# courtois-neuromod/phantom_vlb

Measured on AMD Instinct MI355X. Metric: clips/sec fine-tune VideoLLaMA2-7B+LoRA->2k-voxel head, 1/2/4/8 MI355X, higher is better.
Workload: dtype bf16; 1 GPU; configs[2]: VideoLLaMA2-7B + LoRA r=16 + 2k-voxel head, bf16; clips_per_gpu=3, global_batch=3, seq_len=2048, frames=12, num_target=2048, weights=random-init, comm=none

## Files before the change

include/vlb.h:

```cpp
#ifndef VLB_H
#define VLB_H

#include <stdint.h>

#ifdef __cplusplus
extern "C" {
#endif
#if defined(__GNUC__) || defined(__clang__)
#pragma GCC visibility push(default)
#endif

#define VLB_OK 0
#define VLB_ERR_INVALID (-1)
#define VLB_ERR_LAUNCH (-2)

#define VLB_ABI_VERSION 2

#define VLB_ACT_NONE 0
#define VLB_ACT_QUICK_GELU 1
#define VLB_ACT_GELU 2
#define VLB_ACT_SILU 3
#define VLB_ACT_SWIGLU_PAIR 4
#define VLB_ACT_SWIGLU_BWD 5

// ... 80 lines not shown
                 float* d_ridge_w, float* d_ridge_b, float* d_ln2_w, float* d_ln2_b, float* d_ln1_w, float* d_ln1_b,
                 float* ws, float* dz_ws, float* dpooled_ws, void* dhidden, int B, int S, int E, int V, float eps,
                 float l2_lambda, float loss_scale, float l2_scale, const int* cu_rows, int total_rows, void* stream);

int vlb_feature_cache_store(const float* pooled_raw, const float* sumw, const int32_t* rows, float* cache_pooled,
                            float* cache_sumw, int B, int E, int n_rows, void* stream);
int vlb_head_fwd_cached(const float* cache_pooled, const float* cache_sumw, const int32_t* rows, const void* ln1_w,
                        const void* ln1_b, const void* ln2_w, const void* ln2_b, const void* ridge_w, const void* ridge_b,
                        const float* y, const float* keep_scale, float* ws, float* pooled_raw, float* sumw, float* zhat,
                        float* ln2_rstd, void* z, float* pred, float* loss_terms, int B, int E, int V, int n_rows, float eps,
                        float l2_lambda, void* stream);
int vlb_head_bwd_cached(const void* ln1_w, const void* ln2_w, const void* ridge_w, const float* y, const float* keep_scale,
                        const float* pooled_raw, const float* sumw, const float* zhat, const float* ln2_rstd, const void* z,
                        const float* pred, float* d_ridge_w, float* d_ridge_b, float* d_ln2_w, float* d_ln2_b, float* d_ln1_w,
                        float* d_ln1_b, float* ws, float* dz_ws, float* dpooled_ws, int B, int E, int V, float eps,
                        float l2_lambda, float loss_scale, float l2_scale, void* stream);

int vlb_lora_down(const void* x, int ldx, const void* A, void* t, int ldt, int M, int K, int R, float scale,
                  float drop_p, const uint32_t* seeds_host, void* stream);
int vlb_lora_merge(const void* W, int ldw, void* Wm, int ldwm, const void* Bt, const void* A, int N, int K, int R, float scale,
                   int row_map, void* stream);
int vlb_lora_dx_masked(const void* u, int ldu, const void* At, int ldat, void* dx, int lddx, int M, int K, int R, float drop_p,
                       const uint32_t* seeds_host, void* stream);
int64_t vlb_wgrad_u_ws_floats(int M, int K);
int vlb_wgrad_skinny_u(const void* G, int ldg, const void* X, int ldx, float* dW, float* ws, int M, int K, float alpha,
                       float beta, const void* Bt, float u_scale, void* u, int ldu, float* u_ws, void* stream);
int vlb_wgrad_skinny_u_multi(const void* G, int ldg, const void* X, int ldx, int M, int nproj, const int* cols, float* const* dW,
                             const void* const* Bt, float* ws, float alpha, float beta, float u_scale, void* u, int ldu,
                             float* u_ws, void* stream);
int vlb_transpose16_scatter(const void* jobs, int n_jobs, void* stream);
int vlb_wgrad_splits(int M);
int vlb_wgrad_skinny(const void* G, int ldg, const void* X, int ldx, float* dW, float* ws, int M, int N, int K,
                     float alpha, float beta, float drop_p, const uint32_t* seeds_host, void* stream);

int vlb_sumsq_ws_floats(void);
int vlb_grad_sumsq(const float* g, int64_t n, float* sumsq, float* ws, void* stream);
int vlb_adamw_step(float* master, void* param_bf16, const float* grad, float* m, float* v, int64_t n, float lr,
                   float beta1, float beta2, float eps, float weight_decay, int step, const float* sumsq,
                   float max_norm, void* stream);
int vlb_grad_accum(float* acc, const float* g, int64_t n, int first, float* sumsq, float* ws, void* stream);
int vlb_grad_accum_bf16(float* acc, const void* g_bf16, int64_t n, int first, float* sumsq, float* ws, void* stream);

int vlb_transpose_pad(const void* in, int ld_in, void* out, int ld_out, int R, int C, int Rpad, void* stream);
int64_t vlb_norm_bwd_ws_floats(int rows, int dim);
int64_t vlb_colsum_ws_floats(int rows, int dim);
int vlb_rmsnorm_bwd_dw(const void* x, const void* dy, void* dw_bf16, float* ws, int rows, int dim, float eps, void* stream);
int64_t vlb_rmsnorm_bwd_full_ws_floats(int rows, int dim);
int vlb_rmsnorm_bwd_full(const void* x, const void* w, const void* dy, const void* dx_in, void* dx, void* dw_bf16, float* ws,
                         int rows, int dim, float eps, void* stream);
int vlb_layernorm_bwd(const void* x, const void* w, const void* b, const void* residual, const void* dy, void* dx, void* dres,
                      void* dw_bf16, void* db_bf16, float* ws, int rows, int dim, float eps, int act, void* stream);
int vlb_act_fwd(const void* x, void* y, int64_t n, int act, void* stream);
int vlb_act_bwd(const void* x, const void* dy, void* dx, int64_t n, int act, void* stream);
int vlb_colsum(const void* x, int ld, void* out_bf16, float* ws, int rows, int dim, void* stream);
int vlb_embed_grad(const void* d_embeds, int ld, const int* tok, const int* beg, const int* rows, int n_tokens, void* dE, int D,
                   void* stream);
int vlb_grad_sumsq_bf16(const void* g, int64_t n, float* sumsq, float* ws, void* stream);
int vlb_adamw_step_g16(float* master, void* param_bf16, const void* grad_bf16, float* m, float* v, int64_t n, float lr,
                       float beta1, float beta2, float eps, float weight_decay, int step, const float* sumsq, float max_norm,
                       void* stream);
int64_t vlb_dwconv3x3_bwd_w_ws_floats(int N, int H, int C);
int vlb_dwconv3x3_bwd_w(const void* x, const void* dy, void* dw9_bf16, float* ws, int N, int H, int W, int C, void* stream);
int vlb_se_bwd_gate(const void* x, const void* dy, const void* s, void* ds, int N, int HW, int C, void* stream);
int vlb_se_bwd_x(const void* dy, const void* s, const void* dpool, void* dx, int N, int HW, int C, void* stream);
int vlb_col2im3d_k2s2p1(const void* dcols, void* dx, int B, int T, int H, int W, int C, void* stream);

// ... 45 lines not shown
```

phantom_vlb_amd/_lib.py:

```python
from __future__ import annotations

import ctypes
import os
from ctypes import c_char_p, c_double, c_float, c_int, c_int64, c_void_p

import torch

_HERE = os.path.dirname(os.path.abspath(__file__))
LIB_PATH = os.environ.get("VLB_LIB") or os.path.join(_HERE, "libvlb.so")
IS_PRODUCT_LIB = os.path.abspath(LIB_PATH) == os.path.join(_HERE, "libvlb.so")

P, I, F, L = c_void_p, c_int, c_float, c_int64

SIGNATURES = {
    "vlb_abi_version": [],
    "vlb_last_error": [],
    "vlb_gemm_bf16": [P, I, P, I, P, I, I, I, I, P, P, I, I, P, I, P, I, I, P],
    "vlb_gemm_bf16_ws": [P, I, P, I, P, I, I, I, I, P, P, I, I, P, I, P, I, I, P, L, P],
    "vlb_gemm_swiglu_save": [P, I, P, I, P, I, P, I, I, I, I, P, I, P, I, I, P, L, P],
    "vlb_gemm_workspace_bytes": [],
    "vlb_gemm_plan": [I, I, I, I, I],
    "vlb_gemm_kernel_choice": [I, I, I, I],
    "vlb_transpose_bf16": [P, P, I, I, P],
    "vlb_attention_fwd": [P, I, P, I, P, I, P, I, P, P, I, I, I, I, I, I, F, P, P],
    "vlb_attention_bwd": [P, I, P, I, P, I, P, I, P, I, P, P, P, I, P, I, P, I, P, P, I, I, I, I, I, I, F, P, I, P],
    "vlb_rmsnorm_fwd": [P, P, P, I, I, F, P],
    "vlb_rmsnorm_bwd": [P, P, P, P, P, I, I, F, P],
    "vlb_layernorm_fwd": [P, P, P, P, P, I, I, F, I, P],
    "vlb_rope_inplace": [P, I, P, P, I, I, I, I, I, P, P],
    "vlb_swiglu_fwd": [P, P, I, I, P],
    "vlb_swiglu_bwd": [P, P, P, I, I, P],
    "vlb_add_bf16": [P, P, P, L, P],
    "vlb_patchify": [P, P, I, I, I, I, I, P],
    "vlb_vit_assemble": [P, P, P, P, I, I, I, P],
    "vlb_drop_cls": [P, P, I, I, I, P],
    "vlb_dwconv3x3": [P, P, P, I, I, I, I, P],
    "vlb_se_pool": [P, P, I, I, I, P],
    "vlb_se_scale": [P, P, P, I, I, I, P],
    "vlb_im2col3d_k2s2p1": [P, P, I, I, I, I, I, P],
    "vlb_splice_embed": [P, P, P, P, P, P, I, I, I, I, L, I, P, P, P],
    "vlb_weight_mask": [P, P, P, P, I, I, I, I, I, I, P],
    "vlb_head_partial_rows": [I],
    "vlb_head_ws_floats": [I, I, I, I],
    "vlb_head_fwd": [P] * 19 + [I, I, I, I, F, F, P, P],
    "vlb_head_bwd": [P] * 24 + [I, I, I, I, F, F, F, F, P, I, P],
    "vlb_feature_cache_store": [P] * 5 + [I, I, I, P],
    "vlb_head_fwd_cached": [P] * 19 + [I, I, I, I, F, F, P],
    "vlb_head_bwd_cached": [P] * 20 + [I, I, I, F, F, F, F, P],
    "vlb_gemm_bf16_masked_pair": [P, I, P, I, P, I, I, I, I, P, I, P, I, F, ctypes.c_uint32, P],
    "vlb_gemm_masked_pair_swiglu_bwd": [P, I, P, I, P, I, P, I, I, I, I, P, I, P, I, F, ctypes.c_uint32, P, L, P],
    "vlb_gemm_bf16_masked_pair_ws": [P, I, P, I, P, I, I, I, I, P, I, P, I, F, ctypes.c_uint32, P, L, P],
    "vlb_wgrad_u_ws_floats": [I, I],
    "vlb_wgrad_skinny_u": [P, I, P, I, P, P, I, I, F, F, P, F, P, I, P, P],
    "vlb_wgrad_skinny_u_multi": [P, I, P, I, I, I, P, P, P, P, F, F, F, P, I, P, P],
    "vlb_transpose16_scatter": [P, I, P],
    "vlb_wgrad_splits": [I],
    "vlb_wgrad_skinny": [P, I, P, I, P, P, I, I, I, F, F, F, P, P],
    "vlb_lora_down": [P, I, P, P, I, I, I, I, F, F, P, P],
    "vlb_lora_merge": [P, I, P, I, P, P, I, I, I, F, I, P],
    "vlb_lora_dx_masked": [P, I, P, I, P, I, I, I, I, F, P, P],
    "vlb_sumsq_ws_floats": [],
    "vlb_grad_sumsq": [P, L, P, P, P],
    "vlb_adamw_step": [P, P, P, P, P, L, F, F, F, F, F, I, P, F, P],
    "vlb_grad_accum": [P, P, L, I, P, P, P],
    "vlb_grad_accum_bf16": [P, P, L, I, P, P, P],
    "vlb_dropout_keep_scale": [P, L, F, ctypes.c_uint32, P],
    "vlb_transpose_pad": [P, I, P, I, I, I, I, P],
    "vlb_norm_bwd_ws_floats": [I, I],
    "vlb_colsum_ws_floats": [I, I],
    "vlb_rmsnorm_bwd_dw": [P, P, P, P, I, I, F, P],
    "vlb_rmsnorm_bwd_full_ws_floats": [I, I],
    "vlb_rmsnorm_bwd_full": [P, P, P, P, P, P, P, I, I, F, P],
    "vlb_layernorm_bwd": [P, P, P, P, P, P, P, P, P, P, I, I, F, I, P],
    "vlb_act_fwd": [P, P, L, I, P],
    "vlb_act_bwd": [P, P, P, L, I, P],
    "vlb_colsum": [P, I, P, P, I, I, P],
    "vlb_embed_grad": [P, I, P, P, P, I, P, I, P],
    "vlb_grad_sumsq_bf16": [P, L, P, P, P],
    "vlb_adamw_step_g16": [P, P, P, P, P, L, F, F, F, F, F, I, P, F, P],
    "vlb_dwconv3x3_bwd_w_ws_floats": [I, I, I],
    "vlb_dwconv3x3_bwd_w": [P, P, P, P, I, I, I, I, P],
    "vlb_se_bwd_gate": [P, P, P, P, I, I, I, P],
    "vlb_se_bwd_x": [P, P, P, P, I, I, I, P],
    "vlb_col2im3d_k2s2p1": [P, P, I, I, I, I, I, P],
    "vlb_quantize_mxfp8": [P, I, P, I, P, I, I, I, P],
    "vlb_transpose_quantize_mxfp8": [P, I, P, I, P, I, I, I, I, P],
    "vlb_quantize_dual_mxfp8": [P, I, P, I, P, I, P, I, P, I, I, I, I, P],
    "vlb_rmsnorm_fwd_mxfp8": [P, P, P, P, I, P, I, I, I, F, P],
    "vlb_swiglu_fwd_mxfp8": [P, P, P, I, P, I, I, I, P],
    "vlb_gemm_mxfp8": [P, I, P, I, P, I, P, I, P, I, I, I, I, P, I, P],
# ... 55 lines not shown
```

phantom_vlb_amd/csrc/lora.hip:

```cpp
#include "common.hpp"

namespace {

__device__ __forceinline__ uint32_t lowbias32(uint32_t x) {
  x ^= x >> 16; x *= 0x7feb352dU; x ^= x >> 15; x *= 0x846ca68bU; x ^= x >> 16;
  return x;
}
__device__ __forceinline__ uint32_t drop_bits_pair(uint32_t seed, int64_t m, int K, int kpair) {
  const uint64_t c = (uint64_t)m * (uint64_t)(K >> 1) + (uint64_t)kpair;
  return lowbias32((uint32_t)c ^ lowbias32((uint32_t)(c >> 32) + seed));
}
__device__ __forceinline__ uint32_t drop_bits_fast(uint32_t key, uint32_t row_base, int kpair) {
  return lowbias32((row_base + (uint32_t)kpair) ^ key);
}

struct Seeds { uint32_t s[8]; uint32_t key[8]; uint32_t fast; };

__device__ __forceinline__ uint32_t drop_bits(const Seeds& sd, int g, int64_t m, int K, int kpair) {
  return sd.fast ? drop_bits_fast(sd.key[g], (uint32_t)m * (uint32_t)(K >> 1), kpair) : drop_bits_pair(sd.s[g], m, K, kpair);
}
__device__ __forceinline__ void keep8(const Seeds& sd, int g, int64_t m, int K, int k0, uint32_t thresh, bool (&keep)[8]) {
#pragma unroll
  for (int q = 0; q < 4; ++q) {
    const uint32_t h = drop_bits(sd, g, m, K, (k0 >> 1) + q);
// ... 126 lines not shown
        }
#pragma unroll
        for (int e = 0; e < 4; ++e) sum[4 * t + e] += d[e] * inv_keep;
      }
    }
    if (live) {
      bf16x8 o0, o1;
#pragma unroll
      for (int e = 0; e < 8; ++e) {
        o0[e] = (bf16)((float)old0[e] + sum[e]);
        o1[e] = (bf16)((float)old1[e] + sum[8 + e]);
      }
      *reinterpret_cast<bf16x8*>(prow + kcol) = o0;
      *reinterpret_cast<bf16x8*>(prow + kcol + 8) = o1;
    }
    old0 = nx0; old1 = nx1;
  }
}

constexpr int WG_COLS = 256;
constexpr int WG_STEP = 32;

typedef short s16x4_t __attribute__((ext_vector_type(4)));
typedef short s16x8_t __attribute__((ext_vector_type(8)));

__device__ __forceinline__ void glds16_l(const void* g, void* l) {
  __builtin_amdgcn_global_load_lds((const void __attribute__((address_space(1)))*)g,
                                   (void __attribute__((address_space(3)))*)l, 16, 0, 0);
}
__device__ __forceinline__ int xsw(int r) { return (r & 3) | (((r >> 3) & 1) << 2); }

struct UProj { int col0[4]; const bf16* bt[3]; float* dW[3]; int n; };

template <int G, bool WITH_U = false>
__global__ __launch_bounds__(256) void wgrad_mfma_kernel(const bf16* __restrict__ Gm, int ldg, const bf16* __restrict__ X,
                                                         int ldx, float* __restrict__ ws, int M, int K,
                                                         int rows_per_split, uint32_t thresh, Seeds seeds,
                                                         UProj up = UProj{}, float* __restrict__ upart = nullptr) {
  constexpr int XT = WG_STEP * WG_COLS * 2;
  constexpr int GT = WG_STEP * 16 * G * 2;
  constexpr int UT = WITH_U ? 2 * 4 * 2 * 4 * 64 * 4 : 0;
  __shared__ __attribute__((aligned(16))) char smem[2 * (XT + GT) + UT];
  const int tid = threadIdx.x, lane = tid & 63;
  const int wave = __builtin_amdgcn_readfirstlane(tid >> 6);
  const int c0 = blockIdx.x * WG_COLS;
  const int r0 = blockIdx.y * rows_per_split, r1 = min(M, r0 + rows_per_split);
  const int fr = lane & 15, fq = lane >> 4, tq = fr >> 2, tp = fr & 3;
  const int N = 16 * G;

  f32x4 acc[G][4];
#pragma unroll
  for (int g = 0; g < G; ++g)
#pragma unroll
    for (int n = 0; n < 4; ++n) acc[g][n] = f32x4{0.f, 0.f, 0.f, 0.f};

  bf16x8 btf[2];
  if constexpr (WITH_U) {
    const int pj = (c0 >= up.col0[1]) + (c0 >= up.col0[2]);
    const int pc0 = up.col0[pj], pn = up.col0[pj + 1] - pc0;
    const bf16* Bt = up.bt[pj];
    Gm += 16 * pj;
#pragma unroll
    for (int ks = 0; ks < 2; ++ks) {
      const int lc = c0 - pc0 + wave * 64 + 32 * ks + 8 * fq;
      btf[ks] = *reinterpret_cast<const bf16x8*>(Bt + (int64_t)fr * pn + min(lc, pn - 8));
      if (lc >= pn) btf[ks] = bf16x8{};
    }
  }
  float* ured = reinterpret_cast<float*>(smem + 2 * (XT + GT));

  const int g_r = tid / (2 * G), g_ch = tid % (2 * G);
  const bool g_mine = tid < WG_STEP * 2 * G;
  auto stage = [&](int buf, int m0, bf16x8& gv) {
    char* xb = smem + buf * (XT + GT);
    gv = bf16x8{};
    if (g_mine && m0 + g_r < r1) gv = *reinterpret_cast<const bf16x8*>(Gm + (int64_t)(m0 + g_r) * ldg + g_ch * 8);
#pragma unroll
    for (int i = 0; i < 4; ++i) {
      const int piece = 4 * i + wave, r = 2 * piece + (lane >> 5), pc = lane & 31;
// ... 65 lines not shown
          for (int j = 0; j < 8; ++j) {
            const uint32_t hsh = (j < 4) == !odd ? hm[j & 3] : ho[j & 3];
            const uint32_t bits = odd ? (hsh >> 16) : (hsh & 0xffffu);
            if (bits < thresh) xm[j] = (bf16)0.f;
          }
        }
        acc[g][n] = __builtin_amdgcn_mfma_f32_16x16x32_bf16(af[g], xm, acc[g][n], 0, 0, 0);
      }
    }
    if constexpr (WITH_U) {
      float* mine = ured + ((cur * 4 + wave) * 2) * 4 * 64;
#pragma unroll
      for (int t = 0; t < 2; ++t) {
        f32x4 ua = f32x4{0.f, 0.f, 0.f, 0.f};
#pragma unroll
        for (int ks = 0; ks < 2; ++ks) ua = __builtin_amdgcn_mfma_f32_16x16x32_bf16(btf[ks], xr[t][ks], ua, 0, 0, 0);
#pragma unroll
        for (int e = 0; e < 4; ++e) mine[(t * 4 + e) * 64 + lane] = ua[e];
      }
    }
    if (st + 1 < nsteps) g_store(cur ^ 1, gnext);
    asm volatile("s_waitcnt vmcnt(0)" ::: "memory");
    __syncthreads();
    if constexpr (WITH_U) {
      const float* base = ured + cur * 4 * 2 * 4 * 64;
#pragma unroll
      for (int q = 0; q < 2; ++q) {
        const int idx = tid + 256 * q;
        float v = 0.f;
#pragma unroll
        for (int w = 0; w < 4; ++w) v += base[w * 2 * 4 * 64 + idx];
        const int l = idx & 63, e = (idx >> 6) & 3, t = idx >> 8;
        const int row = m0 + 16 * t + (l & 15), rank = 4 * (l >> 4) + e;
        if (row < r1) upart[((int64_t)blockIdx.x * M + row) * 16 + rank] = v;
      }
    }
  }
#pragma unroll
  for (int g = 0; g < G; ++g)
#pragma unroll
    for (int n = 0; n < 4; ++n) {
      const int col = c0 + wave * 64 + n * 16 + fr;
      if (col < K) {
#pragma unroll
        for (int e = 0; e < 4; ++e) ws[((int64_t)blockIdx.y * N + 16 * g + 4 * fq + e) * K + col] = acc[g][n][e];
      }
    }
}

__global__ void wgrad_reduce_kernel(const float* __restrict__ ws, float* __restrict__ dW, int splits, int64_t nk, float alpha,
                                    float beta) {
  for (int64_t i = blockIdx.x * (int64_t)blockDim.x + threadIdx.x; i < nk; i += (int64_t)gridDim.x * blockDim.x) {
    float s = 0.f;
#pragma unroll 8
    for (int k = 0; k < splits; ++k) s += ws[(int64_t)k * nk + i];
    dW[i] = alpha * s + (beta != 0.f ? beta * dW[i] : 0.f);
  }
}

struct ScatterJob { const bf16* src; bf16* dst; int n; int n0; int ld; int il; };

__global__ __launch_bounds__(256) void transpose16_scatter_kernel(const ScatterJob* __restrict__ jobs) {
  const ScatterJob j = jobs[blockIdx.x];
  const int i = j.n0 + threadIdx.x;
  if (i >= j.n) return;
  bf16x8 lo, hi;
#pragma unroll
  for (int r = 0; r < 8; ++r) {
    lo[r] = j.src[(int64_t)r * j.n + i];
    hi[r] = j.src[(int64_t)(r + 8) * j.n + i];
  }
  bf16* d = j.dst + (int64_t)(j.il ? ((i >> 4) * 32 + (i & 15)) : i) * j.ld;
  *reinterpret_cast<bf16x8*>(d) = lo;
  *reinterpret_cast<bf16x8*>(d + 8) = hi;
}

__global__ void wgrad_u_reduce_kernel(const float* __restrict__ ws, int splits, int K, float alpha, float beta, int wblocks,
                                      const float* __restrict__ upart, bf16* __restrict__ u, int ldu, int M, float scale, UProj up) {
  const int64_t nk = (int64_t)16 * K;
  if ((int)blockIdx.x < wblocks) {
    for (int64_t i = blockIdx.x * (int64_t)blockDim.x + threadIdx.x; i < nk; i += (int64_t)wblocks * blockDim.x) {
      float s = 0.f;
#pragma unroll 8
      for (int k = 0; k < splits; ++k) s += ws[(int64_t)k * nk + i];
      const int r = (int)(i / K), col = (int)(i - (int64_t)r * K);
// ... 116 lines not shown
  return t > 65535u ? 65535u : t;
}
}

extern "C" int vlb_wgrad_splits(int M) {
  if (M >= 4096) return 32;
  int s = (M + 255) / 256;
  return s < 1 ? 1 : s;
}

extern "C" int vlb_wgrad_skinny(const void* G, int ldg, const void* X, int ldx, float* dW, float* ws, int M, int N, int K,
                                float alpha, float beta, float drop_p, const uint32_t* seeds_host, void* stream) {
  VLB_REQUIRE(G && X && dW && ws, "wgrad_skinny: null operand");
  VLB_REQUIRE(M > 0 && (N == 16 || N == 32 || N == 48) && K >= 8 && K % 8 == 0 && ldx % 8 == 0 && ldg % 8 == 0,
              "wgrad_skinny: bad shape M=%d N=%d K=%d (N must be 16, 32 or 48)", M, N, K);
  VLB_REQUIRE(drop_p >= 0.f && drop_p < 1.f && (drop_p == 0.f || seeds_host), "wgrad_skinny: bad dropout arguments");
  VLB_REQUIRE((((uintptr_t)G | (uintptr_t)X) % 16) == 0, "wgrad_skinny: operands must be 16-byte aligned");
  hipStream_t st = as_stream(stream);
  const int splits = vlb_wgrad_splits(M);
  const int rps = (((M + splits - 1) / splits) + WG_STEP - 1) / WG_STEP * WG_STEP;
  const float inv_keep = 1.f / (1.f - drop_p);
  const Seeds sd = make_seeds(seeds_host, N / 16, M, K);
  dim3 grid((K + WG_COLS - 1) / WG_COLS, splits);
  const uint32_t th = thresh16(drop_p);
  switch (N / 16) {
    case 1: hipLaunchKernelGGL(wgrad_mfma_kernel<1>, grid, dim3(256), 0, st, (const bf16*)G, ldg, (const bf16*)X, ldx, ws, M, K, rps, th, sd); break;
    case 2: hipLaunchKernelGGL(wgrad_mfma_kernel<2>, grid, dim3(256), 0, st, (const bf16*)G, ldg, (const bf16*)X, ldx, ws, M, K, rps, th, sd); break;
    default: hipLaunchKernelGGL(wgrad_mfma_kernel<3>, grid, dim3(256), 0, st, (const bf16*)G, ldg, (const bf16*)X, ldx, ws, M, K, rps, th, sd); break;
  }
  VLB_LAUNCH_CHECK();
  const int64_t nk = (int64_t)N * K;
  int blocks = (int)((nk + 255) / 256); if (blocks > 1024) blocks = 1024;
  hipLaunchKernelGGL(wgrad_reduce_kernel, dim3(blocks), dim3(256), 0, st, ws, dW, splits, nk, alpha * inv_keep, beta);
  VLB_LAUNCH_CHECK();
  return VLB_OK;
}

extern "C" int vlb_lora_down(const void* x, int ldx, const void* A, void* t, int ldt, int M, int K, int R, float scale,
                             float drop_p, const uint32_t* seeds_host, void* stream) {
  VLB_REQUIRE(x && A && t, "lora_down: null operand");
  VLB_REQUIRE(M > 0 && K % 32 == 0 && R % 16 == 0 && R >= 16 && R <= 48 && ldx % 8 == 0 && ldt % 4 == 0,
              "lora_down: bad shape M=%d K=%d R=%d", M, K, R);
  VLB_REQUIRE(drop_p >= 0.f && drop_p < 1.f && (drop_p == 0.f || seeds_host), "lora_down: bad dropout arguments");
  const Seeds s = make_seeds(seeds_host, R / 16, M, K);
  const float sc = scale / (1.f - drop_p);
  dim3 grid((M + 16 * LD_RT - 1) / (16 * LD_RT));
  hipStream_t st = as_stream(stream);
  const uint32_t th = thresh16(drop_p);
  switch (R / 16) {
    case 1: hipLaunchKernelGGL(lora_down_kernel<1>, grid, dim3(64 * LD_WAVES), 0, st, (const bf16*)x, ldx, (const bf16*)A, (bf16*)t, ldt, M, K, sc, th, s); break;
    case 2: hipLaunchKernelGGL(lora_down_kernel<2>, grid, dim3(64 * LD_WAVES), 0, st, (const bf16*)x, ldx, (const bf16*)A, (bf16*)t, ldt, M, K, sc, th, s); break;
    default: hipLaunchKernelGGL(lora_down_kernel<3>, grid, dim3(64 * LD_WAVES), 0, st, (const bf16*)x, ldx, (const bf16*)A, (bf16*)t, ldt, M, K, sc, th, s); break;
  }
  VLB_LAUNCH_CHECK();
  return VLB_OK;
}

extern "C" int vlb_lora_dx_masked(const void* u, int ldu, const void* At, int ldat, void* dx, int lddx, int M, int K, int R,
                                  float drop_p, const uint32_t* seeds_host, void* stream) {
  VLB_REQUIRE(u && At && dx, "lora_dx_masked: null operand");
  VLB_REQUIRE(M > 0 && K % 64 == 0 && R % 16 == 0 && R >= 16 && R <= 48 && ldu % 8 == 0 && lddx % 8 == 0 && ldat % 8 == 0 && ldat >= R &&
                  ((uintptr_t)dx % 16) == 0,
              "lora_dx_masked: bad shape M=%d K=%d R=%d", M, K, R);
  VLB_REQUIRE(drop_p >= 0.f && drop_p < 1.f && (drop_p == 0.f || seeds_host), "lora_dx_masked: bad dropout arguments");
  const Seeds s = make_seeds(seeds_host, R / 16, M, K);
  dim3 grid((K + 1023) / 1024, (M + 15) / 16);
// ... 95 lines not shown
```

phantom_vlb_amd/lora.py:

```python
from __future__ import annotations

import ctypes
import math

import torch

from . import ops
from ._lib import check, lib
from .geometry import Geometry, decoder_linears
from .ops import _stream

BF16 = torch.bfloat16
PAD = 64
FUSE_SWIGLU_BWD = True
MERGE_DB_U = True


def _seeds(vals):
    return (ctypes.c_uint32 * len(vals))(*[v & 0xFFFFFFFF for v in vals])


def lora_down(x, A, R, scale, p, seeds, out):
    M, K = x.shape
    check(lib.vlb_lora_down(x.data_ptr(), x.stride(0), A.data_ptr(), out.data_ptr(), out.stride(0), M, K, R, scale, p,
                            _seeds(seeds) if p > 0 else None, _stream()), "vlb_lora_down")
    return out


def lora_dx_masked(u, At, dx, R, p, seeds):
    M, K = dx.shape
    check(lib.vlb_lora_dx_masked(u.data_ptr(), u.stride(0), At.data_ptr(), At.stride(0), dx.data_ptr(), dx.stride(0), M, K, R, p,
                                 _seeds(seeds), _stream()), "vlb_lora_dx_masked")


def wgrad_skinny_u(G, X, dW, ws, Bt, u_scale, u_out, u_ws, alpha=1.0, beta=0.0):
    M, K = X.shape
    check(lib.vlb_wgrad_skinny_u(G.data_ptr(), G.stride(0), X.data_ptr(), X.stride(0), dW.data_ptr(), ws.data_ptr(), M, K,
                                 alpha, beta, Bt.data_ptr(), u_scale, u_out.data_ptr(), u_out.stride(0), u_ws.data_ptr(),
                                 _stream()), "vlb_wgrad_skinny_u")


def wgrad_skinny_u_multi(G, X, cols, dWs, Bts, ws, u_scale, u_out, u_ws, alpha=1.0, beta=0.0):
    M = X.shape[0]
    n = len(cols)
    check(lib.vlb_wgrad_skinny_u_multi(G.data_ptr(), G.stride(0), X.data_ptr(), X.stride(0), M, n, (ctypes.c_int * n)(*cols),
                                       (ctypes.c_void_p * n)(*[t.data_ptr() for t in dWs]), (ctypes.c_void_p * n)(*[t.data_ptr() for t in Bts]),
                                       ws.data_ptr(), alpha, beta, u_scale, u_out.data_ptr(), u_out.stride(0), u_ws.data_ptr(), _stream()),
          "vlb_wgrad_skinny_u_multi")


def wgrad_skinny(G, X, dW, ws, N, alpha=1.0, beta=0.0, p=0.0, seeds=None):
    M, K = X.shape
    check(lib.vlb_wgrad_skinny(G.data_ptr(), G.stride(0), X.data_ptr(), X.stride(0), dW.data_ptr(), ws.data_ptr(), M, N, K,
                               alpha, beta, p, _seeds(seeds) if p > 0 else None, _stream()), "vlb_wgrad_skinny")


GROUPS = (
    ("qkv", ("self_attn.q_proj", "self_attn.k_proj", "self_attn.v_proj")),
    ("o", ("self_attn.o_proj",)),
    ("gu", ("mlp.gate_proj", "mlp.up_proj")),
    ("down", ("mlp.down_proj",)),
)


class LoraState:
    def __init__(self, g: Geometry, weights, r: int, alpha: int, dropout: float, device, seed: int = 1234,
                 sd: dict | None = None, target_modules=None):
        if not isinstance(r, int) or not 1 <= r <= 64:
            raise NotImplementedError(f"lora_r={r}: ranks 1..64 are built (up to four 16-wide MFMA tiles per adapted projection); "
                                      "the reference's setting is 16 (config/experiment/VLB_vllama2_friends_lora.yaml:27)")
        want = sorted(t.split(".")[-1] for _, ts in GROUPS for t in ts)
        if target_modules is not None and sorted(target_modules) != want:
            raise NotImplementedError(f"LoRA target_modules {sorted(target_modules)}: the adapted decoder is built for "
                                      f"exactly {want}")
        self.g, self.w, self.r, self.dev = g, weights, r, device
        self.gu_il = "wgu_il" in weights.layers[0]
        self.c = c = (r + 15) // 16
        self.rp = rp = 16 * c
        self.scale = alpha / r
        self.p = float(dropout)
        self.step = 0
        self.rank = 0
        self.grad_hook = None
        self.base_seed = seed
        self.out_dims = {lin.suffix: lin.out for lin in decoder_linears(g)}
        self.in_dims = {lin.suffix: lin.inp for lin in decoder_linears(g)}
        gen = torch.Generator(device="cpu").manual_seed(seed + 17)
# ... 116 lines not shown
                row += n
            one("o", 0, lw["wo"], mw["wo"])
            if self.gu_il:
                one("gu", 0, lw["wgu_il"], mw["wgu_il"], ops.MERGE_GATE)
                one("gu", 1, lw["wgu_il"], mw["wgu_il"], ops.MERGE_UP)
            else:
                one("gu", 0, lw["wgu"][:g.ff], mw["wgu"][:g.ff])
                one("gu", 1, lw["wgu"][g.ff:], mw["wgu"][g.ff:])
            one("down", 0, lw["wdown"], mw["wdown"])
        self._merged_version = self.version
        return self._merged

    def state_dict(self):
        r = self.r
        return {n: (t[:r].t().contiguous() if "lora_B" in n else t[:r].clone()) for n, t in self.master.items()}

    def load_state_dict(self, sd: dict):
        r = self.r
        for n, t in self.master.items():
            src = sd[n].to(self.dev, torch.float32)
            t[:r].copy_(src.t() if "lora_B" in n else src)
        self.refresh(from_master=True)

    def _seed(self, layer, target_idx):
        x = (self.base_seed * 0x9E3779B1 + self.step * 0x85EBCA6B + layer * 0xC2B2AE35 + target_idx * 0x27D4EB2F
             + self.rank * 0x7F4A7C15) & 0xFFFFFFFF
        return x or 1

    def _workspace(self, M):
        if self._ws is None or self._ws["cap"] < M:
            g, d = self.g, self.dev
            kmax = max(g.ff, g.dim, g.q_dim)
            kgrp = max(2 * g.ff, g.q_dim + 2 * g.kv_dim)
            self._ws = dict(cap=M, wg=torch.empty(lib.vlb_wgrad_splits(M) * 48 * kmax, dtype=torch.float32, device=d),
                            uws=torch.empty(lib.vlb_wgrad_u_ws_floats(M, kgrp), dtype=torch.float32, device=d),
                            u_full=torch.zeros(M, self._rpad_max(), dtype=BF16, device=d))
        self._ws["u"] = self._ws["u_full"][:M]
        return self._ws

    def _rpad_max(self):
        return max(blk["Rpad"] for blk in self.layers[0].values())

    def _group_seeds(self, seeds, n_targets):
        return None if seeds is None else [seeds[j] for j in range(n_targets) for _ in range(self.c)]

    def _t_buffer(self, li, gi, M):
        if getattr(self, "_t_cap", 0) < M:
            self._t_cap = M
            self._t_bufs = torch.zeros(len(self.layers), len(GROUPS), M, self._rpad_max(), dtype=BF16, device=self.dev)
        return self._t_bufs[li, gi, :M, :self.layers[li][GROUPS[gi][0]]["Rpad"]]

    def _lora_t(self, x, blk, seeds, slot=None, p=None):
        t = self._t_buffer(*slot, x.shape[0]) if slot is not None else torch.zeros(x.shape[0], blk["Rpad"], dtype=BF16, device=self.dev)
        p = self.p if p is None else p
        gs = self._group_seeds(seeds, len(blk["targets"])) if p > 0 else None
        for r0 in range(0, blk["R"], 48):
            n = min(48, blk["R"] - r0)
            lora_down(x, blk["A"][r0:r0 + n], n, self.scale, p, None if gs is None else gs[r0 // 16:(r0 + n) // 16], t[:, r0:])
        return t

    def _adapted(self, x, W, blk, seeds, residual=None, slot=None, p=None):
        t = self._lora_t(x, blk, seeds, slot, p)
        return ops.gemm(x, W, residual=residual, a2=t, w2=blk["Bpad"]), t

    def _adapted_mlp_in(self, x, lw, blk, seeds, slot, p=None, save=True):
        if self.gu_il:
            t = self._lora_t(x, blk, seeds, slot, p)
            if save:
                hh, gu = ops.gemm_swiglu_save(x, lw["wgu_il"], a2=t, w2_il=blk["Bpad"])
                return hh, gu, t
# ... 3 lines not shown

    def forward(self, backbone, vision_f32, ids, layout=None, train=True):
        g = self.g
        B = vision_f32.shape[0]
        vid = backbone.video_tokens(vision_f32)
        x, key_mask = backbone.splice(ids, vid, layout)
        return self.decoder_forward(backbone, x, key_mask, B, layout, train=train)

    def decoder_forward(self, backbone, x, key_mask, B, layout=None, train=True):
        g, w = self.g, self.w
        p = None if train else 0.0
        if train:
            self.saved = []
            self.step += 1
        for li, lay in enumerate(self.layers):
            lw = backbone.layer_weights(li)
            sd = [self._seed(li, k) for k in range(7)] if train else [None] * 7
            h1 = ops.rmsnorm(x, lw["in_norm"], g.rms_eps)
            qkv, t_qkv = self._adapted(h1, lw["wqkv"], lay["qkv"], sd[0:3], slot=(li, 0), p=p)
            att = backbone.attention(qkv, key_mask, B, layout, need_lse=train)
            a, lse = att if train else (att, None)
            x2, t_o = self._adapted(a, lw["wo"], lay["o"], sd[3:4], residual=x, slot=(li, 1), p=p)
            h2 = ops.rmsnorm(x2, lw["post_norm"], g.rms_eps)
            hh, gu, t_gu = self._adapted_mlp_in(h2, lw, lay["gu"], sd[4:6], (li, 2), p=p, save=train)
            x3, t_d = self._adapted(hh, lw["wdown"], lay["down"], sd[6:7], residual=x2, slot=(li, 3), p=p)
            if train:
                self.saved.append(dict(x=x, h1=h1, qkv=qkv, a=a, lse=lse, x2=x2, h2=h2, gu=gu, hh=hh, t_qkv=t_qkv, t_o=t_o,
                                       t_gu=t_gu, t_d=t_d, seeds=sd))
            x = x3
        if train:
            self.x_last, self.key_mask, self.B, self.layout = x, key_mask, B, layout
        return ops.rmsnorm(x, w.final_norm, g.rms_eps), key_mask

    def _group_backward(self, li, gname, dy, x_in, t, seeds, W_t, need_dx, swiglu_gu=None):
        lay = self.layers[li][gname]
        ws = self._workspace(dy.shape[0])
        u = ws["u"]
        col = 0
        u = u[:, :lay["Rpad"]]
        rp = self.rp
        names = [f"model.layers.{li}.{tname}" for tname in lay["targets"]]
        cols = [self.out_dims[tname] for tname in lay["targets"]]
        multi = MERGE_DB_U and self.c == 1 and len(cols) > 1 and all(n % 256 == 0 for n in cols) and dy.shape[1] == sum(cols)
        if multi:
            wgrad_skinny_u_multi(t, dy, cols, [self.grads[f"{pre}.lora_B.weight"] for pre in names],
                                 [self.bt[f"{pre}.lora_B.weight"] for pre in names], ws["wg"], self.scale, u, ws["uws"])
        for j, tname in enumerate(() if multi else lay["targets"]):
            n = self.out_dims[tname]
            pre = f"model.layers.{li}.{tname}"
            dyj = dy[:, col:col + n]
            for b in range(self.c):
                k = rp * j + 16 * b
                wgrad_skinny_u(t[:, k:k + 16], dyj, self.grads[f"{pre}.lora_B.weight"][16 * b:16 * b + 16], ws["wg"],
                               self.bt[f"{pre}.lora_B.weight"][16 * b:16 * b + 16], self.scale, u[:, k:k + 16], ws["uws"])
            col += n
        gs = self._group_seeds(seeds, len(lay["targets"])) if self.p > 0 else None
        for r0 in range(0, lay["R"], 48):
            n = min(48, lay["R"] - r0)
            wgrad_skinny(u[:, r0:], x_in, self.grad_A[li][gname][r0:r0 + n], ws["wg"], n, p=self.p,
                         seeds=None if gs is None else gs[r0 // 16:(r0 + n) // 16])
        if not need_dx:
            return None
        if self.p == 0.0:
            dx = ops.gemm(dy, W_t, a2=u, w2=lay["At"])
        elif lay["R"] == 16 and ops.gemm_masked_pair_ok(dy.shape[0], W_t.shape[0], dy.shape[1]):
            if swiglu_gu is not None and FUSE_SWIGLU_BWD:
                return ops.gemm_masked_pair_swiglu_bwd(dy, W_t, swiglu_gu, u, lay["At"], self.p, seeds[0])
            dx = ops.gemm_masked_pair(dy, W_t, u, lay["At"], self.p, seeds[0])
        else:
            dx = ops.gemm(dy, W_t)
            for r0 in range(0, lay["R"], 48):
                n = min(48, lay["R"] - r0)
                lora_dx_masked(u[:, r0:], lay["At"][:, r0:], dx, n, self.p, gs[r0 // 16:(r0 + n) // 16])
        return dx if swiglu_gu is None else ops.swiglu_bwd(swiglu_gu, dx)

    def backward(self, backbone, dhidden):
        g, w = self.g, self.w
        B, layout = self.B, self.layout
        dx = ops.rmsnorm_bwd(self.x_last, w.final_norm, dhidden, g.rms_eps)
        delta = torch.empty(B, g.heads, g.max_len, dtype=torch.float32, device=self.dev)
        for li in range(g.layers - 1, -1, -1):
            lw, sv = backbone.layer_weights(li, transposed=True, direction=-1), self.saved[li]
            sd = sv["seeds"]
            d_gu = self._group_backward(li, "down", dx, sv["hh"], sv["t_d"], sd[6:7], lw["wdown_t"], True, swiglu_gu=sv["gu"])
            d_h2 = self._group_backward(li, "gu", d_gu, sv["h2"], sv["t_gu"], sd[4:6], lw["wgu_t"], True)
            dx2 = ops.rmsnorm_bwd(sv["x2"], lw["post_norm"], d_h2, g.rms_eps, dx_in=dx)
            d_a = self._group_backward(li, "o", dx2, sv["a"], sv["t_o"], sd[3:4], lw["wo_t"], True)
            dqkv = backbone.attention_bwd(sv["qkv"], sv["a"], d_a, sv["lse"], self.key_mask, B, layout, delta)
            need_dx = li > 0
            d_h1 = self._group_backward(li, "qkv", dqkv, sv["h1"], sv["t_qkv"], sd[0:3], lw["wqkv_t"], need_dx)
            if need_dx:
                dx = ops.rmsnorm_bwd(sv["x"], lw["in_norm"], d_h1, g.rms_eps, dx_in=dx2)
            if self.grad_hook is not None:
                self.grad_hook(li)
        self.saved = []
```

Before: 14.87 clips/s.

## Batch per-layer LoRA A-gradient wgrads into one grouped multi-problem launch

Defers the four LoRA A-weight gradient skinny GEMMs in each layer (down, gate/up, o, qkv) and runs them together in one grouped MFMA kernel plus one grouped split-K reduction, instead of separate launches per group. The aim is to cut launch overhead and fill the GPU better, since each individual skinny wgrad has few column blocks. To make this work, the u buffer becomes per-group so the deferred inputs stay valid, and the workspace grows to hold all problems' split-K slabs at once. The cost is more workspace memory and a dispatch switch inside the kernel on each problem's G.

Result: no change. 14.93 clips/s (median of 6 runs) (+0.4%).

```diff
diff --git a/include/vlb.h b/include/vlb.h
--- a/include/vlb.h
+++ b/include/vlb.h
@@ -136,6 +136,9 @@
 int vlb_wgrad_splits(int M);
 int vlb_wgrad_skinny(const void* G, int ldg, const void* X, int ldx, float* dW, float* ws, int M, int N, int K,
                      float alpha, float beta, float drop_p, const uint32_t* seeds_host, void* stream);
+int vlb_wgrad_skinny_multi(int nprob, const void* const* G, const int* ldg, const void* const* X, const int* ldx, const int* N,
+                           const int* K, float* const* dW, float* ws, const int64_t* ws_off, int M, float alpha, float beta,
+                           float drop_p, const uint32_t* seeds_host, void* stream);
 
 int vlb_sumsq_ws_floats(void);
 int vlb_grad_sumsq(const float* g, int64_t n, float* sumsq, float* ws, void* stream);
diff --git a/phantom_vlb_amd/_lib.py b/phantom_vlb_amd/_lib.py
--- a/phantom_vlb_amd/_lib.py
+++ b/phantom_vlb_amd/_lib.py
@@ -56,6 +56,7 @@
     "vlb_transpose16_scatter": [P, I, P],
     "vlb_wgrad_splits": [I],
     "vlb_wgrad_skinny": [P, I, P, I, P, P, I, I, I, F, F, F, P, P],
+    "vlb_wgrad_skinny_multi": [I, P, P, P, P, P, P, P, P, P, I, F, F, F, P, P],
     "vlb_lora_down": [P, I, P, P, I, I, I, I, F, F, P, P],
     "vlb_lora_merge": [P, I, P, I, P, P, I, I, I, F, I, P],
     "vlb_lora_dx_masked": [P, I, P, I, P, I, I, I, I, F, P, P],
diff --git a/phantom_vlb_amd/csrc/lora.hip b/phantom_vlb_amd/csrc/lora.hip
--- a/phantom_vlb_amd/csrc/lora.hip
+++ b/phantom_vlb_amd/csrc/lora.hip
@@ -182,19 +182,21 @@
 
 struct UProj { int col0[4]; const bf16* bt[3]; float* dW[3]; int n; };
 
-template <int G, bool WITH_U = false>
-__global__ __launch_bounds__(256) void wgrad_mfma_kernel(const bf16* __restrict__ Gm, int ldg, const bf16* __restrict__ X,
-                                                         int ldx, float* __restrict__ ws, int M, int K,
-                                                         int rows_per_split, uint32_t thresh, Seeds seeds,
-                                                         UProj up = UProj{}, float* __restrict__ upart = nullptr) {
-  constexpr int XT = WG_STEP * WG_COLS * 2;
-  constexpr int GT = WG_STEP * 16 * G * 2;
-  constexpr int UT = WITH_U ? 2 * 4 * 2 * 4 * 64 * 4 : 0;
-  __shared__ __attribute__((aligned(16))) char smem[2 * (XT + GT) + UT];
+constexpr int WG_XT = WG_STEP * WG_COLS * 2;
+constexpr int wg_gt(int G) { return WG_STEP * 16 * G * 2; }
+constexpr int wg_smem(int G, bool with_u) { return 2 * (WG_XT + wg_gt(G)) + (with_u ? 2 * 4 * 2 * 4 * 64 * 4 : 0); }
+
+template <int G, bool WITH_U>
+__device__ __forceinline__ void wgrad_mfma_block(char* smem, const unsigned bx, const unsigned by, const bf16* __restrict__ Gm, int ldg,
+                                                 const bf16* __restrict__ X, int ldx, float* __restrict__ ws, int M, int K,
+                                                 int rows_per_split, uint32_t thresh, const Seeds& seeds, const UProj& up,
+                                                 float* __restrict__ upart) {
+  constexpr int XT = WG_XT;
+  constexpr int GT = wg_gt(G);
   const int tid = threadIdx.x, lane = tid & 63;
   const int wave = __builtin_amdgcn_readfirstlane(tid >> 6);
-  const int c0 = blockIdx.x * WG_COLS;
-  const int r0 = blockIdx.y * rows_per_split, r1 = min(M, r0 + rows_per_split);
+  const int c0 = bx * WG_COLS;
+  const int r0 = by * rows_per_split, r1 = min(M, r0 + rows_per_split);
   const int fr = lane & 15, fq = lane >> 4, tq = fr >> 2, tp = fr & 3;
   const int N = 16 * G;
 
@@ -326,7 +328,7 @@
         for (int w = 0; w < 4; ++w) v += base[w * 2 * 4 * 64 + idx];
         const int l = idx & 63, e = (idx >> 6) & 3, t = idx >> 8;
         const int row = m0 + 16 * t + (l & 15), rank = 4 * (l >> 4) + e;
-        if (row < r1) upart[((int64_t)blockIdx.x * M + row) * 16 + rank] = v;
+        if (row < r1) upart[((int64_t)bx * M + row) * 16 + rank] = v;
       }
     }
   }
@@ -337,14 +339,61 @@
       const int col = c0 + wave * 64 + n * 16 + fr;
       if (col < K) {
 #pragma unroll
-        for (int e = 0; e < 4; ++e) ws[((int64_t)blockIdx.y * N + 16 * g + 4 * fq + e) * K + col] = acc[g][n][e];
-      }
-    }
+        for (int e = 0; e < 4; ++e) ws[((int64_t)by * N + 16 * g + 4 * fq + e) * K + col] = acc[g][n][e];
+      }
+    }
+}
+
+template <int G, bool WITH_U = false>
+__global__ __launch_bounds__(256) void wgrad_mfma_kernel(const bf16* __restrict__ Gm, int ldg, const bf16* __restrict__ X,
+                                                         int ldx, float* __restrict__ ws, int M, int K,
+                                                         int rows_per_split, uint32_t thresh, Seeds seeds,
+                                                         UProj up = UProj{}, float* __restrict__ upart = nullptr) {
+  __shared__ __attribute__((aligned(16))) char smem[wg_smem(G, WITH_U)];
+  wgrad_mfma_block<G, WITH_U>(smem, blockIdx.x, blockIdx.y, Gm, ldg, X, ldx, ws, M, K, rows_per_split, thresh, seeds, up, upart);
+}
+
+constexpr int WG_MAXP = 4;
+struct WgProb { const bf16* g; const bf16* x; float* ws; int ldg, ldx, K, G; Seeds seeds; };
+struct WgMulti { WgProb p[WG_MAXP]; int cb0[WG_MAXP + 1]; };
+
+__global__ __launch_bounds__(256) void wgrad_mfma_multi_kernel(WgMulti mp, int M, int splits, int rows_per_split, uint32_t thresh) {
+  __shared__ __attribute__((aligned(16))) char smem[wg_smem(3, false)];
+  const int b = blockIdx.x;
+  const int j = (b >= mp.cb0[1] * splits) + (b >= mp.cb0[2] * splits) + (b >= mp.cb0[3] * splits);
+  const WgProb& P = mp.p[j];
+  const int loc = b - mp.cb0[j] * splits, cbn = mp.cb0[j + 1] - mp.cb0[j];
+  const unsigned by = loc / cbn, bx = loc - by * cbn;
+  const UProj none{};
+  switch (P.G) {
+    case 1: wgrad_mfma_block<1, false>(smem, bx, by, P.g, P.ldg, P.x, P.ldx, P.ws, M, P.K, rows_per_split, thresh, P.seeds, none, nullptr); break;
+    case 2: wgrad_mfma_block<2, false>(smem, bx, by, P.g, P.ldg, P.x, P.ldx, P.ws, M, P.K, rows_per_split, thresh, P.seeds, none, nullptr); break;
+    default: wgrad_mfma_block<3, false>(smem, bx, by, P.g, P.ldg, P.x, P.ldx, P.ws, M, P.K, rows_per_split, thresh, P.seeds, none, nullptr); break;
+  }
 }
 
 __global__ void wgrad_reduce_kernel(const float* __restrict__ ws, float* __restrict__ dW, int splits, int64_t nk, float alpha,
                                     float beta) {
   for (int64_t i = blockIdx.x * (int64_t)blockDim.x + threadIdx.x; i < nk; i += (int64_t)gridDim.x * blockDim.x) {
+    float s = 0.f;
+#pragma unroll 8
+    for (int k = 0; k < splits; ++k) s += ws[(int64_t)k * nk + i];
+    dW[i] = alpha * s + (beta != 0.f ? beta * dW[i] : 0.f);
+  }
+}
+
+struct WgRedMulti { const float* ws[WG_MAXP]; float* dW[WG_MAXP]; int64_t start[WG_MAXP + 1]; };
+
+__global__ void wgrad_reduce_multi_kernel(WgRedMulti r, int splits, float alpha, float beta) {
+  const int64_t total = r.start[WG_MAXP];
+  for (int64_t t = blockIdx.x * (int64_t)blockDim.x + threadIdx.x; t < total; t += (int64_t)gridDim.x * blockDim.x) {
+    const float* ws = r.ws[0];
+    float* dW = r.dW[0];
+    int64_t s0 = 0, nk = r.start[1];
+#pragma unroll
+    for (int j = 1; j < WG_MAXP; ++j)
+      if (t >= r.start[j]) { ws = r.ws[j]; dW = r.dW[j]; s0 = r.start[j]; nk = r.start[j + 1] - r.start[j]; }
+    const int64_t i = t - s0;
     float s = 0.f;
 #pragma unroll 8
     for (int k = 0; k < splits; ++k) s += ws[(int64_t)k * nk + i];
@@ -527,6 +576,50 @@
   const int64_t nk = (int64_t)N * K;
   int blocks = (int)((nk + 255) / 256); if (blocks > 1024) blocks = 1024;
   hipLaunchKernelGGL(wgrad_reduce_kernel, dim3(blocks), dim3(256), 0, st, ws, dW, splits, nk, alpha * inv_keep, beta);
+  VLB_LAUNCH_CHECK();
+  return VLB_OK;
+}
+
+extern "C" int vlb_wgrad_skinny_multi(int nprob, const void* const* G, const int* ldg, const void* const* X, const int* ldx,
+                                      const int* N, const int* K, float* const* dW, float* ws, const int64_t* ws_off, int M,
+                                      float alpha, float beta, float drop_p, const uint32_t* seeds_host, void* stream) {
+  VLB_REQUIRE(nprob >= 1 && nprob <= WG_MAXP && G && ldg && X && ldx && N && K && dW && ws && ws_off && M > 0,
+              "wgrad_skinny_multi: bad arguments (1..%d problems, M=%d)", WG_MAXP, M);
+  VLB_REQUIRE(drop_p >= 0.f && drop_p < 1.f && (drop_p == 0.f || seeds_host), "wgrad_skinny_multi: bad dropout arguments");
+  const int splits = vlb_wgrad_splits(M);
+  WgMulti mp{};
+  WgRedMulti rd{};
+  int cb = 0, sg = 0;
+  int64_t el = 0;
+  for (int j = 0; j < nprob; ++j) {
+    VLB_REQUIRE(G[j] && X[j] && dW[j], "wgrad_skinny_multi: problem %d: null operand", j);
+    VLB_REQUIRE((N[j] == 16 || N[j] == 32 || N[j] == 48) && K[j] >= 8 && K[j] % 8 == 0 && ldx[j] % 8 == 0 && ldg[j] % 8 == 0,
+                "wgrad_skinny_multi: problem %d: bad shape N=%d K=%d (N must be 16, 32 or 48)", j, N[j], K[j]);
+    VLB_REQUIRE((((uintptr_t)G[j] | (uintptr_t)X[j]) % 16) == 0 && ws_off[j] >= 0,
+                "wgrad_skinny_multi: problem %d: operands must be 16-byte aligned, the workspace offset >= 0", j);
+    const int64_t nk = (int64_t)N[j] * K[j];
+    for (int i = 0; i < j; ++i) {
+      const int64_t ni = (int64_t)N[i] * K[i] * splits, nj = nk * splits;
+      VLB_REQUIRE(ws_off[i] + ni <= ws_off[j] || ws_off[j] + nj <= ws_off[i], "wgrad_skinny_multi: workspaces of problems %d and %d overlap", i, j);
+    }
+    WgProb& p = mp.p[j];
+    p.g = (const bf16*)G[j]; p.x = (const bf16*)X[j]; p.ws = ws + ws_off[j];
+    p.ldg = ldg[j]; p.ldx = ldx[j]; p.K = K[j]; p.G = N[j] / 16;
+    p.seeds = make_seeds(drop_p > 0.f ? seeds_host + sg : nullptr, N[j] / 16, M, K[j]);
+    sg += N[j] / 16;
+    mp.cb0[j] = cb;
+    cb += (K[j] + WG_COLS - 1) / WG_COLS;
+    rd.ws[j] = p.ws; rd.dW[j] = dW[j]; rd.start[j] = el;
+    el += nk;
+  }
+  for (int j = nprob; j <= WG_MAXP; ++j) { mp.cb0[j] = cb; rd.start[j] = el; }
+  for (int j = nprob; j < WG_MAXP; ++j) { mp.p[j] = mp.p[0]; rd.ws[j] = rd.ws[0]; rd.dW[j] = rd.dW[0]; }
+  hipStream_t st = as_stream(stream);
+  const int rps = (((M + splits - 1) / splits) + WG_STEP - 1) / WG_STEP * WG_STEP;
+  hipLaunchKernelGGL(wgrad_mfma_multi_kernel, dim3(cb * splits), dim3(256), 0, st, mp, M, splits, rps, thresh16(drop_p));
+  VLB_LAUNCH_CHECK();
+  int blocks = (int)((el + 255) / 256); if (blocks > 1024 * nprob) blocks = 1024 * nprob;
+  hipLaunchKernelGGL(wgrad_reduce_multi_kernel, dim3(blocks), dim3(256), 0, st, rd, splits, alpha * (1.f / (1.f - drop_p)), beta);
   VLB_LAUNCH_CHECK();
   return VLB_OK;
 }
diff --git a/phantom_vlb_amd/lora.py b/phantom_vlb_amd/lora.py
--- a/phantom_vlb_amd/lora.py
+++ b/phantom_vlb_amd/lora.py
@@ -14,6 +14,7 @@
 PAD = 64
 FUSE_SWIGLU_BWD = True
 MERGE_DB_U = True
+BATCH_DA_WGRAD = True
 
 
 def _seeds(vals):
@@ -53,6 +54,23 @@
     M, K = X.shape
     check(lib.vlb_wgrad_skinny(G.data_ptr(), G.stride(0), X.data_ptr(), X.stride(0), dW.data_ptr(), ws.data_ptr(), M, N, K,
                                alpha, beta, p, _seeds(seeds) if p > 0 else None, _stream()), "vlb_wgrad_skinny")
+
+
+def wgrad_skinny_multi(problems, ws, alpha=1.0, beta=0.0, p=0.0):
+    n, M = len(problems), problems[0][1].shape[0]
+    offs, off = [], 0
+    for _, X, _, N, _ in problems:
+        offs.append(off)
+        off += lib.vlb_wgrad_splits(M) * N * X.shape[1]
+    assert off <= ws.numel() and all(X.shape[0] == M for _, X, _, _, _ in problems)
+    ptrs = lambda ts: (ctypes.c_void_p * n)(*[t.data_ptr() for t in ts])
+    ints = lambda vs: (ctypes.c_int * n)(*vs)
+    seeds = _seeds([sd for _, _, _, _, sds in problems for sd in sds]) if p > 0 else None
+    check(lib.vlb_wgrad_skinny_multi(n, ptrs([q[0] for q in problems]), ints([q[0].stride(0) for q in problems]),
+                                     ptrs([q[1] for q in problems]), ints([q[1].stride(0) for q in problems]),
+                                     ints([q[3] for q in problems]), ints([q[1].shape[1] for q in problems]),
+                                     ptrs([q[2] for q in problems]), ws.data_ptr(), (ctypes.c_int64 * n)(*offs), M, alpha, beta, p,
+                                     seeds, _stream()), "vlb_wgrad_skinny_multi")
 
 
 GROUPS = (
@@ -235,10 +253,11 @@
             g, d = self.g, self.dev
             kmax = max(g.ff, g.dim, g.q_dim)
             kgrp = max(2 * g.ff, g.q_dim + 2 * g.kv_dim)
-            self._ws = dict(cap=M, wg=torch.empty(lib.vlb_wgrad_splits(M) * 48 * kmax, dtype=torch.float32, device=d),
+            slabs = max(48 * kmax, sum(blk["R"] * blk["A"].shape[1] for blk in self.layers[0].values()))
+            self._ws = dict(cap=M, wg=torch.empty(lib.vlb_wgrad_splits(M) * slabs, dtype=torch.float32, device=d),
                             uws=torch.empty(lib.vlb_wgrad_u_ws_floats(M, kgrp), dtype=torch.float32, device=d),
-                            u_full=torch.zeros(M, self._rpad_max(), dtype=BF16, device=d))
-        self._ws["u"] = self._ws["u_full"][:M]
+                            u_full=torch.zeros(len(GROUPS), M, self._rpad_max(), dtype=BF16, device=d))
+        self._ws["u"] = self._ws["u_full"][:, :M]
         return self._ws
 
     def _rpad_max(self):
@@ -308,10 +327,10 @@
             self.x_last, self.key_mask, self.B, self.layout = x, key_mask, B, layout
         return ops.rmsnorm(x, w.final_norm, g.rms_eps), key_mask
 
-    def _group_backward(self, li, gname, dy, x_in, t, seeds, W_t, need_dx, swiglu_gu=None):
+    def _group_backward(self, li, gname, dy, x_in, t, seeds, W_t, need_dx, swiglu_gu=None, da_batch=None):
         lay = self.layers[li][gname]
         ws = self._workspace(dy.shape[0])
-        u = ws["u"]
+        u = ws["u"][[g[0] for g in GROUPS].index(gname)]
         col = 0
         u = u[:, :lay["Rpad"]]
         rp = self.rp
@@ -331,7 +350,9 @@
                                self.bt[f"{pre}.lora_B.weight"][16 * b:16 * b + 16], self.scale, u[:, k:k + 16], ws["uws"])
             col += n
         gs = self._group_seeds(seeds, len(lay["targets"])) if self.p > 0 else None
-        for r0 in range(0, lay["R"], 48):
+        if da_batch is not None:
+            da_batch.append((u, x_in, self.grad_A[li][gname], lay["R"], gs))
+        for r0 in range(0, lay["R"] if da_batch is None else 0, 48):
             n = min(48, lay["R"] - r0)
             wgrad_skinny(u[:, r0:], x_in, self.grad_A[li][gname][r0:r0 + n], ws["wg"], n, p=self.p,
                          seeds=None if gs is None else gs[r0 // 16:(r0 + n) // 16])
@@ -355,18 +376,22 @@
         B, layout = self.B, self.layout
         dx = ops.rmsnorm_bwd(self.x_last, w.final_norm, dhidden, g.rms_eps)
         delta = torch.empty(B, g.heads, g.max_len, dtype=torch.float32, device=self.dev)
+        batch_da = BATCH_DA_WGRAD and all(blk["R"] <= 48 for blk in self.layers[0].values())
         for li in range(g.layers - 1, -1, -1):
             lw, sv = backbone.layer_weights(li, transposed=True, direction=-1), self.saved[li]
             sd = sv["seeds"]
-            d_gu = self._group_backward(li, "down", dx, sv["hh"], sv["t_d"], sd[6:7], lw["wdown_t"], True, swiglu_gu=sv["gu"])
-            d_h2 = self._group_backward(li, "gu", d_gu, sv["h2"], sv["t_gu"], sd[4:6], lw["wgu_t"], True)
+            da = [] if batch_da else None
+            d_gu = self._group_backward(li, "down", dx, sv["hh"], sv["t_d"], sd[6:7], lw["wdown_t"], True, swiglu_gu=sv["gu"], da_batch=da)
+            d_h2 = self._group_backward(li, "gu", d_gu, sv["h2"], sv["t_gu"], sd[4:6], lw["wgu_t"], True, da_batch=da)
             dx2 = ops.rmsnorm_bwd(sv["x2"], lw["post_norm"], d_h2, g.rms_eps, dx_in=dx)
-            d_a = self._group_backward(li, "o", dx2, sv["a"], sv["t_o"], sd[3:4], lw["wo_t"], True)
+            d_a = self._group_backward(li, "o", dx2, sv["a"], sv["t_o"], sd[3:4], lw["wo_t"], True, da_batch=da)
             dqkv = backbone.attention_bwd(sv["qkv"], sv["a"], d_a, sv["lse"], self.key_mask, B, layout, delta)
             need_dx = li > 0
-            d_h1 = self._group_backward(li, "qkv", dqkv, sv["h1"], sv["t_qkv"], sd[0:3], lw["wqkv_t"], need_dx)
+            d_h1 = self._group_backward(li, "qkv", dqkv, sv["h1"], sv["t_qkv"], sd[0:3], lw["wqkv_t"], need_dx, da_batch=da)
             if need_dx:
                 dx = ops.rmsnorm_bwd(sv["x"], lw["in_norm"], d_h1, g.rms_eps, dx_in=dx2)
+            if batch_da:
+                wgrad_skinny_multi(sorted(da, key=lambda q: -q[3]), self._ws["wg"], p=self.p)
             if self.grad_hook is not None:
                 self.grad_hook(li)
         self.saved = []
```
